# yuxng/PoseCNN

Hardware: NVIDIA H100
Metric: frames/sec on 640x480 RGB, 21 classes, batch 32 (VGG16 + Hough + ROI pose head) (higher is better)
Workload: dtype bf16 operands / fp32 accumulate (conv stack, 1x1 heads), fp16 operands / fp32 accumulate (fc6-fc8), fp32 / int32 elsewhere

## Files before the change

### posecnn_b200/csrc/conv_tc.cu

```cuda
#include <cuda.h>
#include <cuda_bf16.h>

#include <type_traits>

#include "common.cuh"
#include "tc_common.cuh"

namespace pcnn {
namespace convtc {

constexpr int kTileH = 8, kTileW = 16;
static_assert(kTileH * kTileW == kTileM, "pixel tile = two wgmma M blocks");
constexpr int kABytes = kTileM * kKC * 2;
constexpr int kConsumers = 256;
constexpr int kProducerWarp = kConsumers / 32;
constexpr int kThreadsConv = kConsumers + 128;
constexpr int kConsumerRegs = 232, kProducerRegs = 40;
constexpr int kThreadsRow = kConsumers + 32;
constexpr int kStageBytes = 16 * 1024;

struct ConvParams {
    int B, H, W, Cin, Cout;
    int taps, ksize;
    int tiles_h, tiles_w, n_tiles_n, total_tiles;
// ... 107 lines not shown
                    uint8_t* sa = smem + stage * Plan::kStage;
                    mbar_arrive_expect_tx(&full[stage], Plan::kStage);
                    tma_load_4d(sa, &map_in, &full[stage], c0, w0 + dx, h0 + dy, img);
                    tma_load_2d(sa + Plan::kABytesT, &map_w, &full[stage], tap * p.Cin + c0, n0);
                    if (++stage == Plan::kStages) { stage = 0; phase ^= 1; }
                }
            }
        }
    } else {
        setmaxnreg_inc<kConsumerRegs>();
        const int wg = warp >> 2, wq = warp & 3;
        const int row = wg * 64 + wq * 16 + (lane >> 2);
        float acc[kMB][BN / 2];
        int stage = 0, obuf = 0;
        uint32_t phase = 0;
        for (int tile = blockIdx.x; tile < p.total_tiles; tile += gridDim.x) {
            const int nt = tile % p.n_tiles_n;
            int rest = tile / p.n_tiles_n;
            const int tw = rest % p.tiles_w; rest /= p.tiles_w;
            const int th = rest % p.tiles_h;
            const int img = rest / p.tiles_h;
            const int h0 = th * p.tile_h, w0 = tw * p.tile_w, n0 = nt * BN;
            int prev = -1;
            for (int ks = 0; ks < ksteps; ks++) {
                mbar_wait(&full[stage], phase);
                const uint32_t sa = smem_u32(smem + stage * Plan::kStage);
                const uint64_t db = make_desc(sa + Plan::kABytesT);
#pragma unroll
                for (int h = 0; h < kMB; h++) acc_fence<BN / 2>(acc[h]);
                wgmma_fence();
#pragma unroll
                for (int h = 0; h < kMB; h++) {
                    const uint64_t da = make_desc(sa + (h * 2 + wg) * 64 * 128);
#pragma unroll
                    for (int k = 0; k < kKC / 16; k++)
                        wgmma<BN, 0, 0, 0>(acc[h], da + (uint64_t)(k * 2), db + (uint64_t)(k * 2), (ks | k) != 0);
                }
                wgmma_commit();
#pragma unroll
                for (int h = 0; h < kMB; h++) acc_fence<BN / 2>(acc[h]);
                if (prev >= 0) {
                    wgmma_wait<1>();
                    release(&empty[prev], lane);
                }
                prev = stage;
                if (++stage == Plan::kStages) { stage = 0; phase ^= 1; }
            }
            wgmma_wait<0>();
#pragma unroll
            for (int h = 0; h < kMB; h++) acc_fence<BN / 2>(acc[h]);
            release(&empty[prev], lane);
#pragma unroll
            for (int h = 0; h < kMB; h++) {
                if (h > 0 && h0 + 8 * h >= p.H) break;
#pragma unroll
                for (int g = 0; g < BN / 64; g++) {
                    if (threadIdx.x == 0) tma_store_wait_read<1>();
                    consumer_sync();
                    uint8_t* ob = out_stage + obuf * kStageBytes;
                    stage_rows(ob, acc[h] + g * 32, p.bias + n0 + g * 64, p.relu, row, lane & 3);
                    if (p.pool) {
                        consumer_sync();
                        pool_staged(ob, threadIdx.x);
                    }
                    fence_proxy_async();
                    consumer_sync();
                    if (threadIdx.x == 0) {
                        if (!p.pool) tma_store_4d(&map_out, ob, n0 + g * 64, w0, h0 + 8 * h, img);
                        else tma_store_4d(&map_out, ob, n0 + g * 64, w0 >> 1, (h0 >> 1) + 4 * h, img);
                        tma_store_commit();
                    }
                    obuf ^= 1;
                }
            }
        }
        if (threadIdx.x == 0) tma_store_wait_all();
    }
}

constexpr int kRowPx = 128, kPatchW = 130, kPatchH = 4;
constexpr int kPatchBytes = kPatchW * kPatchH * 128;
constexpr int kRowAStages = 2;

template <int BN, bool RESB>
struct RowPlan {
    static constexpr int kBBytes = BN * 128;
    static constexpr int kBStages = RESB ? 9 : 6;
    static constexpr int kBOff = kRowAStages * kPatchBytes;
    static constexpr int kOutOff = kBOff + kBStages * kBBytes;
    static constexpr int kOutBytes = RESB ? kStageBytes : 2 * kStageBytes;
    static constexpr int kBarOff = kOutOff + kOutBytes;
    static constexpr int kTotal = kBarOff + 256 + 1024;
};

template <int BN, bool RESB>
__global__ void __launch_bounds__(kThreadsRow, 1)
k_conv_row2(const __grid_constant__ CUtensorMap map_in , const __grid_constant__ CUtensorMap map_w,
            const __grid_constant__ CUtensorMap map_out ,
            const ConvParams p)
{
    using Plan = RowPlan<BN, RESB>;
    static_assert(BN == 64, "row mode: 64-channel N tiles");
    extern __shared__ uint8_t smem_raw[];
    uint8_t* smem = reinterpret_cast<uint8_t*>((reinterpret_cast<uintptr_t>(smem_raw) + 1023) & ~(uintptr_t)1023);
    uint8_t* sB = smem + Plan::kBOff;
    uint8_t* out_stage = smem + Plan::kOutOff;
    uint64_t* fullA = reinterpret_cast<uint64_t*>(smem + Plan::kBarOff);
    uint64_t* emptyA = fullA + kRowAStages;
    uint64_t* fullB = emptyA + kRowAStages;
    uint64_t* emptyB = fullB + Plan::kBStages;
    uint64_t* wbar = emptyB + Plan::kBStages;
    const int warp = threadIdx.x >> 5, lane = threadIdx.x & 31;
    const int kchunks = p.Cin / kKC;
    const int tile0 = RESB ? blockIdx.x / p.n_tiles_n : blockIdx.x;
    const int tstep = RESB ? gridDim.x / p.n_tiles_n : gridDim.x;
    const int tcount = RESB ? p.total_tiles / p.n_tiles_n : p.total_tiles;
    const int nt_fixed = blockIdx.x % p.n_tiles_n;
    if (warp == kProducerWarp && lane == 0) {
        asm volatile("prefetch.tensormap [%0];" ::"l"(&map_in) : "memory");
        asm volatile("prefetch.tensormap [%0];" ::"l"(&map_w) : "memory");
        asm volatile("prefetch.tensormap [%0];" ::"l"(&map_out) : "memory");
        for (int s = 0; s < kRowAStages; s++) { mbar_init(&fullA[s], 1); mbar_init(&emptyA[s], kConsumers / 32); }
        for (int s = 0; s < Plan::kBStages; s++) { mbar_init(&fullB[s], 1); mbar_init(&emptyB[s], kConsumers / 32); }
        mbar_init(wbar, 1);
        fence_barrier_init();
    }
    __syncthreads();

    if (warp == kProducerWarp) {
        if (elect_one()) {
            int sa = 0, sb = 0;
            uint32_t pa = 0, pb = 0;
            if (RESB) {
                mbar_arrive_expect_tx(wbar, 9 * Plan::kBBytes);
                for (int tap = 0; tap < 9; tap++)
                    tma_load_2d(sB + tap * Plan::kBBytes, &map_w, wbar, tap * p.Cin, nt_fixed * BN);
            }
            for (int tile = tile0; tile < tcount; tile += tstep) {
                const int nt = RESB ? nt_fixed : tile % p.n_tiles_n;
                int rest = RESB ? tile : tile / p.n_tiles_n;
                const int tw = rest % p.tiles_w; rest /= p.tiles_w;
                const int yp = rest % p.tiles_h;
                const int img = rest / p.tiles_h;
                const int y0 = 2 * yp, x0 = tw * kRowPx, n0 = nt * BN;
                for (int c = 0; c < kchunks; c++) {
                    mbar_wait(&emptyA[sa], pa ^ 1);
                    mbar_arrive_expect_tx(&fullA[sa], kPatchBytes);
                    tma_load_4d(smem + sa * kPatchBytes, &map_in, &fullA[sa], c * kKC, x0 - 1, y0 - 1, img);
                    if (++sa == kRowAStages) { sa = 0; pa ^= 1; }
                    if (!RESB) {
                        for (int tap = 0; tap < 9; tap++) {
                            mbar_wait(&emptyB[sb], pb ^ 1);
                            mbar_arrive_expect_tx(&fullB[sb], Plan::kBBytes);
                            tma_load_2d(sB + sb * Plan::kBBytes, &map_w, &fullB[sb], tap * p.Cin + c * kKC, n0);
                            if (++sb == Plan::kBStages) { sb = 0; pb ^= 1; }
                        }
                    }
                }
            }
        }
    } else {
        constexpr int kH = BN / 2;
        const int wg = warp >> 2, wq = warp & 3;
        const int row = wg * 64 + wq * 16 + (lane >> 2);
        float acc[2 * kH];
        int sa = 0, sb = 0, obuf = 0;
        uint32_t pa = 0, pb = 0;
        if (RESB) mbar_wait(wbar, 0);
        for (int tile = tile0; tile < tcount; tile += tstep) {
            const int nt = RESB ? nt_fixed : tile % p.n_tiles_n;
            int rest = RESB ? tile : tile / p.n_tiles_n;
            const int tw = rest % p.tiles_w; rest /= p.tiles_w;
            const int yp = rest % p.tiles_h;
            const int img = rest / p.tiles_h;
            const int y0 = 2 * yp, x0 = tw * kRowPx, n0 = nt * BN;
            for (int c = 0; c < kchunks; c++) {
                mbar_wait(&fullA[sa], pa);
                const uint32_t a_base = smem_u32(smem + sa * kPatchBytes) + wg * 64 * 128;
                if constexpr (RESB) {
                    acc_fence<2 * kH>(acc);
                    wgmma_fence();
#pragma unroll
                    for (int o = 0; o < 4; o++) {
                        const int rho = o == 0 ? 1 : (o == 1 ? 2 : (o == 2 ? 0 : 3));
#pragma unroll
                        for (int s3 = 0; s3 < 3; s3++) {
                            const uint64_t da = make_desc(a_base + (uint32_t)((rho * kPatchW + s3) * 128));
#pragma unroll
                            for (int j = 0; j < 2; j++) {
                                const int r = rho - j;
                                if (r < 0 || r > 2) continue;
                                const uint64_t db = make_desc(smem_u32(sB + (r * 3 + s3) * Plan::kBBytes));
#pragma unroll
                                for (int k = 0; k < kKC / 16; k++)
                                    wgmma<BN, 0, 0, 0>(acc + j * kH, da + (uint64_t)(k * 2), db + (uint64_t)(k * 2), (c | o | s3 | k) != 0);
                            }
                        }
                    }
                    wgmma_commit();
                    wgmma_wait<0>();
                    acc_fence<2 * kH>(acc);
                } else {
                    int prevb = -1;
                    for (int tap = 0; tap < 9; tap++) {
                        mbar_wait(&fullB[sb], pb);
                        const int r = tap / 3, s = tap - 3 * r;
                        const uint64_t db = make_desc(smem_u32(sB + sb * Plan::kBBytes));
                        acc_fence<2 * kH>(acc);
                        wgmma_fence();
#pragma unroll
                        for (int j = 0; j < 2; j++) {
                            const uint64_t da = make_desc(a_base + (uint32_t)(((r + j) * kPatchW + s) * 128));
#pragma unroll
                            for (int k = 0; k < kKC / 16; k++)
                                wgmma<BN, 0, 0, 0>(acc + j * kH, da + (uint64_t)(k * 2), db + (uint64_t)(k * 2), (c | tap | k) != 0);
                        }
                        wgmma_commit();
                        acc_fence<2 * kH>(acc);
                        if (prevb >= 0) {
                            wgmma_wait<1>();
                            release(&emptyB[prevb], lane);
                        }
                        prevb = sb;
                        if (++sb == Plan::kBStages) { sb = 0; pb ^= 1; }
                    }
                    wgmma_wait<0>();
                    acc_fence<2 * kH>(acc);
                    release(&emptyB[prevb], lane);
                }
                release(&emptyA[sa], lane);
                if (++sa == kRowAStages) { sa = 0; pa ^= 1; }
            }
            if (!p.pool) {
#pragma unroll
                for (int j = 0; j < 2; j++) {
#pragma unroll
                    for (int g = 0; g < BN / 64; g++) {
                        if (threadIdx.x == 0) { if (RESB) tma_store_wait_read<0>(); else tma_store_wait_read<1>(); }
                        consumer_sync();
                        uint8_t* ob = out_stage + (RESB ? 0 : obuf * kStageBytes);
                        stage_rows(ob, acc + j * kH + g * 32, p.bias + n0 + g * 64, p.relu, row, lane & 3);
                        fence_proxy_async();
                        consumer_sync();
                        if (threadIdx.x == 0) {
                            tma_store_4d(&map_out, ob, n0 + g * 64, x0, y0 + j, img);
                            tma_store_commit();
                        }
                        obuf ^= 1;
                    }
                }
            } else {
#pragma unroll
                for (int g = 0; g < BN / 64; g++) {
                    if (threadIdx.x == 0) tma_store_wait_read<1>();
                    consumer_sync();
                    uint8_t* ob = out_stage + obuf * (RESB ? kStageBytes / 2 : kStageBytes);
                    const float* a0 = acc + g * 32;
                    const float* a1 = acc + kH + g * 32;
                    const float* bias = p.bias + n0 + g * 64;
                    const int q = lane & 3;
#pragma unroll
                    for (int i = 0; i < 2; i++) {
                        const int r = row + 8 * i;
                        const int prow = r >> 1;
#pragma unroll
                        for (int jj = 0; jj < 8; jj++) {
                            const int c = 8 * jj + 2 * q;
                            float v0 = fmaxf(a0[4 * jj + 2 * i], a1[4 * jj + 2 * i]) + __ldg(bias + c);
                            float v1 = fmaxf(a0[4 * jj + 2 * i + 1], a1[4 * jj + 2 * i + 1]) + __ldg(bias + c + 1);
                            if (p.relu) { v0 = fmaxf(v0, 0.f); v1 = fmaxf(v1, 0.f); }
                            uint32_t pk = pack_bf16(v0, v1);
                            uint32_t o1 = __shfl_xor_sync(0xffffffffu, pk, 4);
                            __nv_bfloat162 m2 = __hmax2(*reinterpret_cast<__nv_bfloat162*>(&pk), *reinterpret_cast<__nv_bfloat162*>(&o1));
                            if ((lane & 4) == 0)
                                *reinterpret_cast<__nv_bfloat162*>(ob + prow * 128 + ((jj ^ (prow & 7)) << 4) + 4 * q) = m2;
                        }
                    }
                    fence_proxy_async();
                    consumer_sync();
                    if (threadIdx.x == 0) {
                        tma_store_4d(&map_out, ob, n0 + g * 64, x0 >> 1, y0 >> 1, img);
                        tma_store_commit();
                    }
                    obuf ^= 1;
                }
            }
        }
        if (threadIdx.x == 0) tma_store_wait_all();
    }
}

constexpr int kC1Stages = 6;
constexpr int kC1EpiGroups = 2, kC1BuildGroups = 4;
constexpr int kC1Threads = 128 * (kC1EpiGroups + kC1BuildGroups);
constexpr int kC1PatchWords = 10 * 16;
constexpr int kC1PatchOff = kC1Stages * kABytes + 64 * 128 + kC1EpiGroups * 2 * kStageBytes;
constexpr int kC1BarOff = kC1PatchOff + kC1BuildGroups * 2 * kC1PatchWords * 4;
constexpr int kC1Smem = kC1BarOff + 256 + 1024;

struct DepthIn { float d; };

__device__ __forceinline__ float depth_gray(float d)
{
    return __fmul_rn(fminf(fmaxf(__fdiv_rn(d, 2000.f), 0.f), 1.f), 255.f);
}

template <typename TIn>
__global__ void __launch_bounds__(kC1Threads, 1)
k_conv1_tc(const TIn* __restrict__ in, const __grid_constant__ CUtensorMap map_w, const __grid_constant__ CUtensorMap map_out,
           const ConvParams p, float m0, float m1, float m2)
{
    constexpr int BN = 64;
    extern __shared__ uint8_t smem_raw[];
    uint8_t* smem = reinterpret_cast<uint8_t*>((reinterpret_cast<uintptr_t>(smem_raw) + 1023) & ~(uintptr_t)1023);
    uint8_t* sb = smem + kC1Stages * kABytes;
    uint8_t* out_stage = sb + 64 * 128;
    uint64_t* full = reinterpret_cast<uint64_t*>(smem + kC1BarOff);
    uint64_t* empty = full + kC1Stages;
    uint64_t* wbar = empty + kC1Stages;
    const int warp = threadIdx.x >> 5, lane = threadIdx.x & 31;

    if (threadIdx.x == 0) {
        asm volatile("prefetch.tensormap [%0];" ::"l"(&map_w) : "memory");
        asm volatile("prefetch.tensormap [%0];" ::"l"(&map_out) : "memory");
        for (int s = 0; s < kC1Stages; s++) { mbar_init(&full[s], 4); mbar_init(&empty[s], 4); }
        mbar_init(wbar, 1);
        fence_barrier_init();
    }
    __syncthreads();

    if (warp >= 4 * kC1EpiGroups) {
        const int group = (threadIdx.x - 128 * kC1EpiGroups) >> 7;
        const int r = (threadIdx.x - 128 * kC1EpiGroups) & 127;
        const int hl = r >> 4, wl = r & 15;
        uint32_t* patch_base = reinterpret_cast<uint32_t*>(smem + kC1PatchOff);
        const bool fast_u8 = sizeof(TIn) == 1 && (p.W & 3) == 0 && (reinterpret_cast<uintptr_t>(in) & 3) == 0;
        int it = 0, lit = 0;
        for (int tile = blockIdx.x; tile < p.total_tiles; tile += gridDim.x, it++) {
            if (it % kC1BuildGroups != group) continue;
            const int stage = it % kC1Stages;
            const uint32_t phase = (it / kC1Stages) & 1;
            const int tw = tile % p.tiles_w;
            const int rest = tile / p.tiles_w;
            const int th = rest % p.tiles_h, img = rest / p.tiles_h;
            const int y = th * kTileH + hl, x = tw * kTileW + wl;
            constexpr int kInCh = std::is_same<TIn, DepthIn>::value ? 1 : 3;
            const TIn* base = in + (size_t)img * p.H * p.W * kInCh;
            float v[32];
            v[27] = 1.f; v[28] = 1.f;
#pragma unroll
            for (int k = 29; k < 32; k++) v[k] = 0.f;
            bool done = false;
            if constexpr (sizeof(TIn) == 1) {
                if (fast_u8) {
                    uint32_t* pw = patch_base + (group * 2 + (lit & 1)) * kC1PatchWords;
                    const int y0 = th * kTileH - 1, wq0 = 12 * tw - 1, row_words = (p.W * 3) >> 2;
                    const uint32_t* img32 = reinterpret_cast<const uint32_t*>(base);
                    for (int idx = r; idx < 140; idx += 128) {
                        const int prow = idx / 14, wi = idx - prow * 14;
                        const int yy = y0 + prow, wq = wq0 + wi;
                        uint32_t word = 0;
                        if (yy >= 0 && yy < p.H && wq >= 0 && wq < row_words) word = __ldg(img32 + (size_t)yy * row_words + wq);
                        pw[prow * 16 + wi] = word;
                    }
                    if (group == 0) asm volatile("bar.sync 3, 128;" ::: "memory");
                    else if (group == 1) asm volatile("bar.sync 4, 128;" ::: "memory");
                    else if (group == 2) asm volatile("bar.sync 5, 128;" ::: "memory");
                    else asm volatile("bar.sync 6, 128;" ::: "memory");
                    const int boff = 1 + 3 * wl, w0 = boff >> 2, o = boff & 3;
                    const uint32_t sel = (uint32_t)(o | ((o + 1) << 4) | ((o + 2) << 8) | ((o + 3) << 12));
                    const bool border = th == 0 || th * kTileH + kTileH + 1 > p.H || tw == 0 || tw * kTileW + kTileW + 1 > p.W;
// ... 203 lines not shown
        if (yy >= 0 && yy < H && xx >= 0 && xx < W) {
            if constexpr (std::is_same<TIn, DepthIn>::value)
                v = __fsub_rn(depth_gray(img[yy * W + xx].d), c == 0 ? m0 : (c == 1 ? m1 : m2));
            else
                v = (float)img[(yy * W + xx) * 3 + c] - (c == 0 ? m0 : (c == 1 ? m1 : m2));
        }
        patch[r][rem] = v;
    }
    __syncthreads();
    const int j = t & 7;
#pragma unroll
    for (int pass = 0; pass < kSeg / 32; pass++) {
        const int xl = pass * 32 + (t >> 3), x = x0 + xl;
        if (x >= W) break;
        __align__(16) __nv_bfloat16 v[8];
#pragma unroll
        for (int e = 0; e < 8; e++) {
            const int k = j * 8 + e;
            float val = 0.f;
            if (k < 27) {
                const int dy = k / 9, rem = k - dy * 9;
                val = patch[dy][xl * 3 + rem];
            }
            v[e] = __float2bfloat16_rn(val);
        }
        *reinterpret_cast<uint4*>(out + (((size_t)n * H + y) * W + x) * 64 + j * 8) = *reinterpret_cast<const uint4*>(v);
    }
}

__global__ void __launch_bounds__(256)
k_maxpool2x2_bf16(const __nv_bfloat16* __restrict__ in, __nv_bfloat16* __restrict__ out, int B, int H, int W, int C)
{
    const int Ho = H / 2, Wo = W / 2, cg = C / 8;
    const size_t total = (size_t)B * Ho * Wo * cg;
    for (size_t idx = (size_t)blockIdx.x * blockDim.x + threadIdx.x; idx < total; idx += (size_t)gridDim.x * blockDim.x) {
        const int g = (int)(idx % cg);
        size_t r = idx / cg;
        const int xo = (int)(r % Wo); r /= Wo;
        const int yo = (int)(r % Ho);
        const size_t n = r / Ho;
        const __nv_bfloat16* p0 = in + ((n * H + 2 * yo) * W + 2 * xo) * C + g * 8;
        uint4 a = __ldg(reinterpret_cast<const uint4*>(p0));
        uint4 b = __ldg(reinterpret_cast<const uint4*>(p0 + C));
        uint4 c = __ldg(reinterpret_cast<const uint4*>(p0 + (size_t)W * C));
        uint4 d = __ldg(reinterpret_cast<const uint4*>(p0 + (size_t)W * C + C));
        uint4 o;
        const __nv_bfloat162* pa = reinterpret_cast<const __nv_bfloat162*>(&a);
        const __nv_bfloat162* pb = reinterpret_cast<const __nv_bfloat162*>(&b);
        const __nv_bfloat162* pc = reinterpret_cast<const __nv_bfloat162*>(&c);
        const __nv_bfloat162* pd = reinterpret_cast<const __nv_bfloat162*>(&d);
        __nv_bfloat162* po = reinterpret_cast<__nv_bfloat162*>(&o);
#pragma unroll
        for (int k = 0; k < 4; k++) po[k] = __hmax2(__hmax2(pa[k], pb[k]), __hmax2(pc[k], pd[k]));
        *reinterpret_cast<uint4*>(out + ((n * Ho + yo) * Wo + xo) * C + g * 8) = o;
    }
}

static int make_map_nhwc(CUtensorMap* m, const void* ptr, int B, int H, int W, int C, int box_c, int box_w = kTileW, int box_h = kTileH)
{
    EncodeTiledFn enc = get_encode();
    if (!enc) { set_error("cuTensorMapEncodeTiled unavailable (driver too old?)"); return PCNN_E_CUDA; }
    cuuint64_t dims[4] = {(cuuint64_t)C, (cuuint64_t)W, (cuuint64_t)H, (cuuint64_t)B};
    cuuint64_t strides[3] = {(cuuint64_t)C * 2, (cuuint64_t)W * C * 2, (cuuint64_t)H * W * C * 2};
    cuuint32_t box[4] = {(cuuint32_t)box_c, (cuuint32_t)box_w, (cuuint32_t)box_h, 1};
    cuuint32_t es[4] = {1, 1, 1, 1};
    CUresult r = enc(m, CU_TENSOR_MAP_DATA_TYPE_BFLOAT16, 4, const_cast<void*>(ptr), dims, strides, box, es,
                     CU_TENSOR_MAP_INTERLEAVE_NONE, CU_TENSOR_MAP_SWIZZLE_128B, CU_TENSOR_MAP_L2_PROMOTION_L2_256B,
                     CU_TENSOR_MAP_FLOAT_OOB_FILL_NONE);
    if (r != CUDA_SUCCESS) { set_error("cuTensorMapEncodeTiled(NHWC %dx%dx%dx%d) failed: %d", B, H, W, C, (int)r); return PCNN_E_CUDA; }
    return PCNN_OK;
}

template <int BN, int BM = kTileM>
static int launch_conv(const CUtensorMap& mi, const CUtensorMap& mw, const CUtensorMap& mo, const ConvParams& p, int num_sms,
                       cudaStream_t st)
{
    using Plan = SmemPlan<BN, BM>;
    PCNN_SMEM_OPTIN((k_conv_tc<BN, BM>), Plan::kTotal, "conv_tc");
    int grid = p.total_tiles < num_sms ? p.total_tiles : num_sms;
    k_conv_tc<BN, BM><<<grid, kThreadsConv, Plan::kTotal, st>>>(mi, mw, mo, p);
    return check_launch("conv_tc");
}

template <int BN, bool RESB>
static int launch_conv_row2(const CUtensorMap& mi, const CUtensorMap& mw, const CUtensorMap& mo, const ConvParams& p, int num_sms,
                            cudaStream_t st)
{
    using Plan = RowPlan<BN, RESB>;
    PCNN_SMEM_OPTIN((k_conv_row2<BN, RESB>), Plan::kTotal, "conv_row2");
    int grid = p.total_tiles < num_sms ? p.total_tiles : num_sms;
    if (RESB) grid = grid / p.n_tiles_n * p.n_tiles_n;
    k_conv_row2<BN, RESB><<<grid, kThreadsRow, Plan::kTotal, st>>>(mi, mw, mo, p);
    return check_launch("conv_row2");
}

}
}

using namespace pcnn;
using namespace pcnn::convtc;

static int conv_bf16_tc_impl(const void* in, const void* weights, const float* bias, void* out, int B, int H, int W, int Cin,
                            int Cout, int ksize, int relu, int block_n, int pool, void* stream);

extern "C" int pcnn_conv_bf16_tc(const void* in, const void* weights, const float* bias, void* out, int B, int H, int W,
                                 int Cin, int Cout, int ksize, int relu, int block_n, void* stream)
{
    return conv_bf16_tc_impl(in, weights, bias, out, B, H, W, Cin, Cout, ksize, relu, block_n, 0, stream);
}

extern "C" int pcnn_conv_pool_bf16_tc(const void* in, const void* weights, const float* bias, void* out_pooled, int B, int H,
                                      int W, int Cin, int Cout, int ksize, int relu, int block_n, void* stream)
{
    PCNN_REQUIRE(H % 2 == 0 && W % 2 == 0, "conv_pool: needs even H, W (got %d x %d)", H, W);
    return conv_bf16_tc_impl(in, weights, bias, out_pooled, B, H, W, Cin, Cout, ksize, relu, block_n, 1, stream);
}

static int conv_bf16_tc_impl(const void* in, const void* weights, const float* bias, void* out, int B, int H, int W, int Cin,
                            int Cout, int ksize, int relu, int block_n, int pool, void* stream)
{
    PCNN_REQUIRE(in && weights && bias && out, "conv: NULL tensor pointer");
    PCNN_REQUIRE(ksize == 1 || ksize == 3, "conv: ksize must be 1 or 3 (got %d)", ksize);
    PCNN_REQUIRE(Cin % 64 == 0 && Cin >= 64, "conv: Cin must be a multiple of 64 (got %d)", Cin);
    PCNN_REQUIRE(Cout % 64 == 0 && Cout >= 64, "conv: Cout must be a multiple of 64 (got %d)", Cout);
    PCNN_REQUIRE(B >= 1 && H >= 1 && W >= 1, "conv: bad shape");
    int bn = block_n;
    if (bn == 0) bn = Cout % 256 == 0 && ksize * ksize * Cin >= 2304 ? 256 : (Cout % 128 == 0 ? 128 : 64);
    PCNN_REQUIRE((bn == 64 || bn == 128 || bn == 256) && Cout % bn == 0, "conv: block_n %d does not divide Cout %d", bn, Cout);
    int dev = 0, sms = kNumSMs;
    cudaGetDevice(&dev);
    cudaDeviceGetAttribute(&sms, cudaDevAttrMultiProcessorCount, dev);
    cudaStream_t st = (cudaStream_t)stream;
    CUtensorMap mi, mw, mo;
    int rc;
    const bool tile256 = block_n == 0 && ksize == 3 && Cin <= 128 && Cout == 128;
    if (block_n == 0 && ksize == 3 && Cin <= 128 && Cout == 64 && H % 2 == 0 && W >= kRowPx) {
        const bool resb = Cin == 64;
        bn = 64;
        rc = make_map_nhwc(&mi, in, B, H, W, Cin, kKC, kPatchW, kPatchH);
        if (rc) return rc;
        rc = make_map_weights(&mw, weights, 9 * Cin, Cout, bn);
        if (rc) return rc;
        rc = pool ? make_map_nhwc(&mo, out, B, H / 2, W / 2, Cout, 64, kRowPx / 2, 1) : make_map_nhwc(&mo, out, B, H, W, Cout, 64, kRowPx, 1);
        if (rc) return rc;
        ConvParams p;
        p.B = B; p.H = H; p.W = W; p.Cin = Cin; p.Cout = Cout; p.ksize = 3; p.taps = 9;
        p.tile_h = 2; p.tile_w = kRowPx;
        p.tiles_h = H / 2;
        p.tiles_w = (W + kRowPx - 1) / kRowPx;
        p.n_tiles_n = Cout / bn;
        p.total_tiles = B * p.tiles_h * p.tiles_w * p.n_tiles_n;
        p.relu = relu; p.pool = pool; p.bias = bias; p.kc_outer = 0;
        if (resb && p.total_tiles >= p.n_tiles_n) return launch_conv_row2<64, true>(mi, mw, mo, p, sms, st);
        return launch_conv_row2<64, false>(mi, mw, mo, p, sms, st);
    }
    int tile_h = kTileH, tile_w = kTileW;
    if (tile256) tile_h = 2 * kTileH;
    else if (!pool && ((H + 15) / 16) * ((W + 7) / 8) < ((H + 7) / 8) * ((W + 15) / 16)) { tile_h = 16; tile_w = 8; }
    rc = make_map_nhwc(&mi, in, B, H, W, Cin, kKC, tile_w, tile_h);
    if (rc) return rc;
    rc = make_map_weights(&mw, weights, ksize * ksize * Cin, Cout, bn);
    if (rc) return rc;
    rc = pool ? make_map_nhwc(&mo, out, B, H / 2, W / 2, Cout, 64, kTileW / 2, kTileH / 2)
              : make_map_nhwc(&mo, out, B, H, W, Cout, 64, tile_w, tile256 ? kTileH : tile_h);
    if (rc) return rc;
    ConvParams p;
    p.B = B; p.H = H; p.W = W; p.Cin = Cin; p.Cout = Cout;
    p.ksize = ksize; p.taps = ksize * ksize;
    p.tile_h = tile_h; p.tile_w = tile_w;
    p.tiles_h = (H + tile_h - 1) / tile_h;
    p.tiles_w = (W + tile_w - 1) / tile_w;
    p.n_tiles_n = Cout / bn;
    p.total_tiles = B * p.tiles_h * p.tiles_w * p.n_tiles_n;
    p.relu = relu;
    p.pool = pool;
    p.bias = bias;
    p.kc_outer = tile256 && H % 2 == 0 && W >= kRowPx;
    if (tile256) return launch_conv<128, 256>(mi, mw, mo, p, sms, st);
    if (bn == 256) return launch_conv<256>(mi, mw, mo, p, sms, st);
    if (bn == 128) return launch_conv<128>(mi, mw, mo, p, sms, st);
    return launch_conv<64>(mi, mw, mo, p, sms, st);
}

extern "C" int pcnn_conv3x3_small_cin(const float* in, const float* weights_hwio, const float* bias, void* out, int B, int H,
                                      int W, int Cin, int Cout, int relu, void* stream)
{
    PCNN_REQUIRE(in && weights_hwio && bias && out, "conv_small: NULL tensor pointer");
    PCNN_REQUIRE(Cin >= 1 && Cin <= 8 && Cout % 16 == 0 && Cout <= 128, "conv_small: needs Cin <= 8, Cout %% 16 == 0, Cout <= 128");
    size_t smem = sizeof(float) * (size_t)(9 * Cin + 1) * Cout;
    size_t total = (size_t)B * H * W * (Cout / 16);
    int blocks = (int)((total + 255) / 256 < (size_t)kNumSMs * 8 ? (total + 255) / 256 : (size_t)kNumSMs * 8);
    k_conv_small_cin<16><<<blocks, 256, smem, (cudaStream_t)stream>>>(in, weights_hwio, bias, (__nv_bfloat16*)out, B, H, W, Cin,
                                                                      Cout, relu);
    return check_launch("conv_small_cin");
}

extern "C" int pcnn_maxpool2x2_bf16(const void* in, void* out, int B, int H, int W, int C, void* stream)
{
    PCNN_REQUIRE(in && out, "maxpool: NULL tensor pointer");
    PCNN_REQUIRE(H % 2 == 0 && W % 2 == 0 && C % 8 == 0, "maxpool: needs even H, W and C %% 8 == 0 (got %d,%d,%d)", H, W, C);
    size_t total = (size_t)B * (H / 2) * (W / 2) * (C / 8);
    int blocks = (int)((total + 255) / 256 < (size_t)kNumSMs * 16 ? (total + 255) / 256 : (size_t)kNumSMs * 16);
    k_maxpool2x2_bf16<<<blocks, 256, 0, (cudaStream_t)stream>>>((const __nv_bfloat16*)in, (__nv_bfloat16*)out, B, H, W, C);
    return check_launch("maxpool2x2");
}

extern "C" int pcnn_im2col_c3(const void* in, int in_is_u8, const float* mean3_host, void* out_bf16, int B, int H, int W,
                              void* stream)
{
    PCNN_REQUIRE(in && out_bf16, "im2col: NULL tensor pointer");
    float m0 = 0.f, m1 = 0.f, m2 = 0.f;
    if (mean3_host) { m0 = mean3_host[0]; m1 = mean3_host[1]; m2 = mean3_host[2]; }
    PCNN_REQUIRE(H <= 65535 && B <= 65535, "im2col: image too tall for the launch grid");
    dim3 grid((W + 127) / 128, H, B);
    cudaStream_t st = (cudaStream_t)stream;
    if (in_is_u8)
        k_im2col_c3<unsigned char><<<grid, 256, 0, st>>>((const unsigned char*)in, (__nv_bfloat16*)out_bf16, H, W, m0, m1, m2);
    else
        k_im2col_c3<float><<<grid, 256, 0, st>>>((const float*)in, (__nv_bfloat16*)out_bf16, H, W, m0, m1, m2);
    return check_launch("im2col_c3");
}

extern "C" int pcnn_im2col_depth(const float* depth, const float* mean3_host, void* out_bf16, int B, int H, int W, void* stream)
{
    PCNN_REQUIRE(depth && out_bf16, "im2col_depth: NULL tensor pointer");
    PCNN_REQUIRE(B >= 1 && H >= 1 && W >= 1, "im2col_depth: bad shape (%d,%d,%d)", B, H, W);
    PCNN_REQUIRE(H <= 65535 && B <= 65535, "im2col_depth: image too tall for the launch grid");
    float m0 = 0.f, m1 = 0.f, m2 = 0.f;
    if (mean3_host) { m0 = mean3_host[0]; m1 = mean3_host[1]; m2 = mean3_host[2]; }
    dim3 grid((W + 127) / 128, H, B);
    k_im2col_c3<DepthIn><<<grid, 256, 0, (cudaStream_t)stream>>>((const DepthIn*)depth, (__nv_bfloat16*)out_bf16, H, W, m0, m1, m2);
    return check_launch("im2col_depth");
}

static int conv1_fused_impl(const void* in, int in_kind, const float* mean3_host, const void* weights_bf16,
                            const float* bias, void* out_bf16, int B, int H, int W, int relu, void* stream);

// ... 46 lines not shown
```

Before: 2887.

## Add swapped-operand row conv kernel with resident weights for Cin=64 layers

Replaces the resident-weight variant of the row conv kernel with a new kernel for Cin=64, Cout=64 3x3 convs. Weights become the wgmma A operand (M=64 output channels) and input pixels the N=128 operand. Two consumer warpgroups each take alternate tiles, with named barriers so their wgmma issue interleaves. The epilogue writes transposed output through half-row TMA stores, with an in-register 2x2 pool path. The goal is wider N per wgmma and overlap of one warpgroup's epilogue with the other's math. The cost is a more complex epilogue with 64-pixel stores and per-warpgroup serialization.

Result: faster. 2969, median of 6 (+2.8%).

```diff
diff --git a/posecnn_b200/csrc/conv_tc.cu b/posecnn_b200/csrc/conv_tc.cu
--- a/posecnn_b200/csrc/conv_tc.cu
+++ b/posecnn_b200/csrc/conv_tc.cu
@@ -213,24 +213,23 @@
 constexpr int kPatchBytes = kPatchW * kPatchH * 128;
 constexpr int kRowAStages = 2;
 
-template <int BN, bool RESB>
+template <int BN>
 struct RowPlan {
     static constexpr int kBBytes = BN * 128;
-    static constexpr int kBStages = RESB ? 9 : 6;
+    static constexpr int kBStages = 6;
     static constexpr int kBOff = kRowAStages * kPatchBytes;
     static constexpr int kOutOff = kBOff + kBStages * kBBytes;
-    static constexpr int kOutBytes = RESB ? kStageBytes : 2 * kStageBytes;
-    static constexpr int kBarOff = kOutOff + kOutBytes;
+    static constexpr int kBarOff = kOutOff + 2 * kStageBytes;
     static constexpr int kTotal = kBarOff + 256 + 1024;
 };
 
-template <int BN, bool RESB>
+template <int BN>
 __global__ void __launch_bounds__(kThreadsRow, 1)
 k_conv_row2(const __grid_constant__ CUtensorMap map_in , const __grid_constant__ CUtensorMap map_w,
             const __grid_constant__ CUtensorMap map_out ,
             const ConvParams p)
 {
-    using Plan = RowPlan<BN, RESB>;
+    using Plan = RowPlan<BN>;
     static_assert(BN == 64, "row mode: 64-channel N tiles");
     extern __shared__ uint8_t smem_raw[];
     uint8_t* smem = reinterpret_cast<uint8_t*>((reinterpret_cast<uintptr_t>(smem_raw) + 1023) & ~(uintptr_t)1023);
@@ -240,20 +239,14 @@
     uint64_t* emptyA = fullA + kRowAStages;
     uint64_t* fullB = emptyA + kRowAStages;
     uint64_t* emptyB = fullB + Plan::kBStages;
-    uint64_t* wbar = emptyB + Plan::kBStages;
     const int warp = threadIdx.x >> 5, lane = threadIdx.x & 31;
     const int kchunks = p.Cin / kKC;
-    const int tile0 = RESB ? blockIdx.x / p.n_tiles_n : blockIdx.x;
-    const int tstep = RESB ? gridDim.x / p.n_tiles_n : gridDim.x;
-    const int tcount = RESB ? p.total_tiles / p.n_tiles_n : p.total_tiles;
-    const int nt_fixed = blockIdx.x % p.n_tiles_n;
     if (warp == kProducerWarp && lane == 0) {
         asm volatile("prefetch.tensormap [%0];" ::"l"(&map_in) : "memory");
         asm volatile("prefetch.tensormap [%0];" ::"l"(&map_w) : "memory");
         asm volatile("prefetch.tensormap [%0];" ::"l"(&map_out) : "memory");
         for (int s = 0; s < kRowAStages; s++) { mbar_init(&fullA[s], 1); mbar_init(&emptyA[s], kConsumers / 32); }
         for (int s = 0; s < Plan::kBStages; s++) { mbar_init(&fullB[s], 1); mbar_init(&emptyB[s], kConsumers / 32); }
-        mbar_init(wbar, 1);
         fence_barrier_init();
     }
     __syncthreads();
@@ -262,14 +255,9 @@
         if (elect_one()) {
             int sa = 0, sb = 0;
             uint32_t pa = 0, pb = 0;
-            if (RESB) {
-                mbar_arrive_expect_tx(wbar, 9 * Plan::kBBytes);
-                for (int tap = 0; tap < 9; tap++)
-                    tma_load_2d(sB + tap * Plan::kBBytes, &map_w, wbar, tap * p.Cin, nt_fixed * BN);
-            }
-            for (int tile = tile0; tile < tcount; tile += tstep) {
-                const int nt = RESB ? nt_fixed : tile % p.n_tiles_n;
-                int rest = RESB ? tile : tile / p.n_tiles_n;
+            for (int tile = blockIdx.x; tile < p.total_tiles; tile += gridDim.x) {
+                const int nt = tile % p.n_tiles_n;
+                int rest = tile / p.n_tiles_n;
                 const int tw = rest % p.tiles_w; rest /= p.tiles_w;
                 const int yp = rest % p.tiles_h;
                 const int img = rest / p.tiles_h;
@@ -279,13 +267,11 @@
                     mbar_arrive_expect_tx(&fullA[sa], kPatchBytes);
                     tma_load_4d(smem + sa * kPatchBytes, &map_in, &fullA[sa], c * kKC, x0 - 1, y0 - 1, img);
                     if (++sa == kRowAStages) { sa = 0; pa ^= 1; }
-                    if (!RESB) {
-                        for (int tap = 0; tap < 9; tap++) {
-                            mbar_wait(&emptyB[sb], pb ^ 1);
-                            mbar_arrive_expect_tx(&fullB[sb], Plan::kBBytes);
-                            tma_load_2d(sB + sb * Plan::kBBytes, &map_w, &fullB[sb], tap * p.Cin + c * kKC, n0);
-                            if (++sb == Plan::kBStages) { sb = 0; pb ^= 1; }
-                        }
+                    for (int tap = 0; tap < 9; tap++) {
+                        mbar_wait(&emptyB[sb], pb ^ 1);
+                        mbar_arrive_expect_tx(&fullB[sb], Plan::kBBytes);
+                        tma_load_2d(sB + sb * Plan::kBBytes, &map_w, &fullB[sb], tap * p.Cin + c * kKC, n0);
+                        if (++sb == Plan::kBStages) { sb = 0; pb ^= 1; }
                     }
                 }
             }
@@ -297,10 +283,9 @@
         float acc[2 * kH];
         int sa = 0, sb = 0, obuf = 0;
         uint32_t pa = 0, pb = 0;
-        if (RESB) mbar_wait(wbar, 0);
-        for (int tile = tile0; tile < tcount; tile += tstep) {
-            const int nt = RESB ? nt_fixed : tile % p.n_tiles_n;
-            int rest = RESB ? tile : tile / p.n_tiles_n;
+        for (int tile = blockIdx.x; tile < p.total_tiles; tile += gridDim.x) {
+            const int nt = tile % p.n_tiles_n;
+            int rest = tile / p.n_tiles_n;
             const int tw = rest % p.tiles_w; rest /= p.tiles_w;
             const int yp = rest % p.tiles_h;
             const int img = rest / p.tiles_h;
@@ -308,57 +293,32 @@
             for (int c = 0; c < kchunks; c++) {
                 mbar_wait(&fullA[sa], pa);
                 const uint32_t a_base = smem_u32(smem + sa * kPatchBytes) + wg * 64 * 128;
-                if constexpr (RESB) {
+                int prevb = -1;
+                for (int tap = 0; tap < 9; tap++) {
+                    mbar_wait(&fullB[sb], pb);
+                    const int r = tap / 3, s = tap - 3 * r;
+                    const uint64_t db = make_desc(smem_u32(sB + sb * Plan::kBBytes));
                     acc_fence<2 * kH>(acc);
                     wgmma_fence();
 #pragma unroll
-                    for (int o = 0; o < 4; o++) {
-                        const int rho = o == 0 ? 1 : (o == 1 ? 2 : (o == 2 ? 0 : 3));
-#pragma unroll
-                        for (int s3 = 0; s3 < 3; s3++) {
-                            const uint64_t da = make_desc(a_base + (uint32_t)((rho * kPatchW + s3) * 128));
-#pragma unroll
-                            for (int j = 0; j < 2; j++) {
-                                const int r = rho - j;
-                                if (r < 0 || r > 2) continue;
-                                const uint64_t db = make_desc(smem_u32(sB + (r * 3 + s3) * Plan::kBBytes));
-#pragma unroll
-                                for (int k = 0; k < kKC / 16; k++)
-                                    wgmma<BN, 0, 0, 0>(acc + j * kH, da + (uint64_t)(k * 2), db + (uint64_t)(k * 2), (c | o | s3 | k) != 0);
-                            }
-                        }
+                    for (int j = 0; j < 2; j++) {
+                        const uint64_t da = make_desc(a_base + (uint32_t)(((r + j) * kPatchW + s) * 128));
+#pragma unroll
+                        for (int k = 0; k < kKC / 16; k++)
+                            wgmma<BN, 0, 0, 0>(acc + j * kH, da + (uint64_t)(k * 2), db + (uint64_t)(k * 2), (c | tap | k) != 0);
                     }
                     wgmma_commit();
-                    wgmma_wait<0>();
                     acc_fence<2 * kH>(acc);
-                } else {
-                    int prevb = -1;
-                    for (int tap = 0; tap < 9; tap++) {
-                        mbar_wait(&fullB[sb], pb);
-                        const int r = tap / 3, s = tap - 3 * r;
-                        const uint64_t db = make_desc(smem_u32(sB + sb * Plan::kBBytes));
-                        acc_fence<2 * kH>(acc);
-                        wgmma_fence();
-#pragma unroll
-                        for (int j = 0; j < 2; j++) {
-                            const uint64_t da = make_desc(a_base + (uint32_t)(((r + j) * kPatchW + s) * 128));
-#pragma unroll
-                            for (int k = 0; k < kKC / 16; k++)
-                                wgmma<BN, 0, 0, 0>(acc + j * kH, da + (uint64_t)(k * 2), db + (uint64_t)(k * 2), (c | tap | k) != 0);
-                        }
-                        wgmma_commit();
-                        acc_fence<2 * kH>(acc);
-                        if (prevb >= 0) {
-                            wgmma_wait<1>();
-                            release(&emptyB[prevb], lane);
-                        }
-                        prevb = sb;
-                        if (++sb == Plan::kBStages) { sb = 0; pb ^= 1; }
-                    }
-                    wgmma_wait<0>();
-                    acc_fence<2 * kH>(acc);
-                    release(&emptyB[prevb], lane);
-                }
+                    if (prevb >= 0) {
+                        wgmma_wait<1>();
+                        release(&emptyB[prevb], lane);
+                    }
+                    prevb = sb;
+                    if (++sb == Plan::kBStages) { sb = 0; pb ^= 1; }
+                }
+                wgmma_wait<0>();
+                acc_fence<2 * kH>(acc);
+                release(&emptyB[prevb], lane);
                 release(&emptyA[sa], lane);
                 if (++sa == kRowAStages) { sa = 0; pa ^= 1; }
             }
@@ -367,9 +327,9 @@
                 for (int j = 0; j < 2; j++) {
 #pragma unroll
                     for (int g = 0; g < BN / 64; g++) {
-                        if (threadIdx.x == 0) { if (RESB) tma_store_wait_read<0>(); else tma_store_wait_read<1>(); }
+                        if (threadIdx.x == 0) tma_store_wait_read<1>();
                         consumer_sync();
-                        uint8_t* ob = out_stage + (RESB ? 0 : obuf * kStageBytes);
+                        uint8_t* ob = out_stage + obuf * kStageBytes;
                         stage_rows(ob, acc + j * kH + g * 32, p.bias + n0 + g * 64, p.relu, row, lane & 3);
                         fence_proxy_async();
                         consumer_sync();
@@ -385,7 +345,7 @@
                 for (int g = 0; g < BN / 64; g++) {
                     if (threadIdx.x == 0) tma_store_wait_read<1>();
                     consumer_sync();
-                    uint8_t* ob = out_stage + obuf * (RESB ? kStageBytes / 2 : kStageBytes);
+                    uint8_t* ob = out_stage + obuf * kStageBytes;
                     const float* a0 = acc + g * 32;
                     const float* a1 = acc + kH + g * 32;
                     const float* bias = p.bias + n0 + g * 64;
@@ -418,6 +378,156 @@
             }
         }
         if (threadIdx.x == 0) tma_store_wait_all();
+    }
+}
+
+constexpr int kRowNWBytes = 64 * 128;
+constexpr int kRowNOutBytes = 64 * 128;
+constexpr int kRowNWOff = kRowAStages * kPatchBytes;
+constexpr int kRowNOutOff = kRowNWOff + 9 * kRowNWBytes;
+constexpr int kRowNBarOff = kRowNOutOff + 2 * kRowNOutBytes;
+constexpr int kRowNSmem = kRowNBarOff + 256 + 1024;
+
+__device__ __forceinline__ void bar_sync(int id, int n) { asm volatile("bar.sync %0, %1;" ::"r"(id), "r"(n) : "memory"); }
+__device__ __forceinline__ void bar_arrive(int id, int n) { asm volatile("bar.arrive %0, %1;" ::"r"(id), "r"(n) : "memory"); }
+
+__global__ void __launch_bounds__(kThreadsConv, 1)
+k_conv_rown(const __grid_constant__ CUtensorMap map_in , const __grid_constant__ CUtensorMap map_w,
+            const __grid_constant__ CUtensorMap map_out ,
+            const ConvParams p)
+{
+    extern __shared__ uint8_t smem_raw[];
+    uint8_t* smem = reinterpret_cast<uint8_t*>((reinterpret_cast<uintptr_t>(smem_raw) + 1023) & ~(uintptr_t)1023);
+    uint8_t* sW = smem + kRowNWOff;
+    uint64_t* fullA = reinterpret_cast<uint64_t*>(smem + kRowNBarOff);
+    uint64_t* emptyA = fullA + kRowAStages;
+    uint64_t* wbar = emptyA + kRowAStages;
+    const int warp = threadIdx.x >> 5, lane = threadIdx.x & 31;
+    if (warp == kProducerWarp && lane == 0) {
+        asm volatile("prefetch.tensormap [%0];" ::"l"(&map_in) : "memory");
+        asm volatile("prefetch.tensormap [%0];" ::"l"(&map_w) : "memory");
+        asm volatile("prefetch.tensormap [%0];" ::"l"(&map_out) : "memory");
+        for (int s = 0; s < kRowAStages; s++) { mbar_init(&fullA[s], 1); mbar_init(&emptyA[s], 4); }
+        mbar_init(wbar, 1);
+        fence_barrier_init();
+    }
+    __syncthreads();
+
+    if (warp >= kProducerWarp) {
+        setmaxnreg_dec<kProducerRegs>();
+        if (warp == kProducerWarp && elect_one()) {
+            mbar_arrive_expect_tx(wbar, 9 * kRowNWBytes);
+            for (int tap = 0; tap < 9; tap++) tma_load_2d(sW + tap * kRowNWBytes, &map_w, wbar, tap * kKC, 0);
+            int it = 0;
+#pragma unroll 1
+            for (int tile = blockIdx.x; tile < p.total_tiles; tile += gridDim.x, it++) {
+                const int tw = tile % p.tiles_w, rest = tile / p.tiles_w;
+                const int yp = rest % p.tiles_h, img = rest / p.tiles_h;
+                const int s = it & 1;
+                mbar_wait(&emptyA[s], ((it >> 1) & 1) ^ 1);
+                mbar_arrive_expect_tx(&fullA[s], kPatchBytes);
+                tma_load_4d(smem + s * kPatchBytes, &map_in, &fullA[s], 0, tw * kRowPx - 1, 2 * yp - 1, img);
+            }
+        }
+    } else {
+        setmaxnreg_inc<kConsumerRegs>();
+        const int wg = warp >> 2, wq = warp & 3, q = lane & 3;
+        const int co = wq * 16 + (lane >> 2);
+        const float bias0 = __ldg(p.bias + co), bias1 = __ldg(p.bias + co + 8);
+        const bool issuer = (threadIdx.x & 127) == 0;
+        uint8_t* ob = smem + kRowNOutOff + wg * kRowNOutBytes;
+        const uint32_t w_base = smem_u32(sW);
+        const uint32_t b_base = smem_u32(smem + wg * kPatchBytes);
+        float acc[2][64];
+        mbar_wait(wbar, 0);
+        int it = wg;
+        for (int tile = blockIdx.x + wg * gridDim.x; tile < p.total_tiles; tile += 2 * gridDim.x, it += 2) {
+            const int tw = tile % p.tiles_w, rest = tile / p.tiles_w;
+            const int yp = rest % p.tiles_h, img = rest / p.tiles_h;
+            const int y0 = 2 * yp, x0 = tw * kRowPx;
+            if (it > 0) bar_sync(3 + wg, 256);
+            mbar_wait(&fullA[wg], (it >> 1) & 1);
+            acc_fence<64>(acc[0]);
+            acc_fence<64>(acc[1]);
+            wgmma_fence();
+#pragma unroll
+            for (int j = 0; j < 2; j++) {
+#pragma unroll
+                for (int ri = 0; ri < 3; ri++) {
+                    const int r = j == 0 ? (ri + 1) % 3 : ri;
+#pragma unroll
+                    for (int s = 0; s < 3; s++) {
+                        const uint64_t da = make_desc(w_base + (uint32_t)((r * 3 + s) * kRowNWBytes));
+                        const uint64_t db = make_desc(b_base + (uint32_t)(((r + j) * kPatchW + s) * 128));
+#pragma unroll
+                        for (int k = 0; k < kKC / 16; k++)
+                            wgmma<128, 0, 0, 0>(acc[j], da + (uint64_t)(k * 2), db + (uint64_t)(k * 2), (ri | s | k) != 0);
+                    }
+                }
+            }
+            wgmma_commit();
+            if (tile + gridDim.x < p.total_tiles) bar_arrive(3 + (wg ^ 1), 256);
+            wgmma_wait<0>();
+            acc_fence<64>(acc[0]);
+            acc_fence<64>(acc[1]);
+            release(&emptyA[wg], lane);
+            if (p.pool) {
+                if (issuer) tma_store_wait_read<0>();
+                bar_sync(1 + wg, 128);
+#pragma unroll
+                for (int jn = 0; jn < 16; jn++) {
+                    const int pp = 4 * jn + q;
+                    float v[2][2];
+#pragma unroll
+                    for (int e = 0; e < 2; e++) {
+                        v[e][0] = fmaxf(acc[0][4 * jn + e], acc[1][4 * jn + e]) + bias0;
+                        v[e][1] = fmaxf(acc[0][4 * jn + 2 + e], acc[1][4 * jn + 2 + e]) + bias1;
+                        if (p.relu) { v[e][0] = fmaxf(v[e][0], 0.f); v[e][1] = fmaxf(v[e][1], 0.f); }
+                    }
+                    uint32_t pe = pack_bf16(v[0][0], v[0][1]), po = pack_bf16(v[1][0], v[1][1]);
+                    __nv_bfloat162 m2 = __hmax2(*reinterpret_cast<__nv_bfloat162*>(&pe), *reinterpret_cast<__nv_bfloat162*>(&po));
+                    uint8_t* rowp = ob + pp * 128 + (lane >> 2) * 2;
+                    *reinterpret_cast<__nv_bfloat16*>(rowp + (((2 * wq) ^ (pp & 7)) << 4)) = m2.x;
+                    *reinterpret_cast<__nv_bfloat16*>(rowp + (((2 * wq + 1) ^ (pp & 7)) << 4)) = m2.y;
+                }
+                fence_proxy_async();
+                bar_sync(1 + wg, 128);
+                if (issuer) {
+                    tma_store_4d(&map_out, ob, 0, x0 >> 1, y0 >> 1, img);
+                    tma_store_commit();
+                }
+            } else {
+#pragma unroll
+                for (int j = 0; j < 2; j++) {
+#pragma unroll
+                    for (int h = 0; h < 2; h++) {
+                        if (x0 + 64 * h >= p.W) continue;
+                        if (issuer) tma_store_wait_read<0>();
+                        bar_sync(1 + wg, 128);
+#pragma unroll
+                        for (int jl = 0; jl < 8; jl++) {
+                            const int jn = 8 * h + jl;
+#pragma unroll
+                            for (int e = 0; e < 2; e++) {
+                                const int pl = 8 * jl + 2 * q + e;
+                                float v0 = acc[j][4 * jn + e] + bias0, v1 = acc[j][4 * jn + 2 + e] + bias1;
+                                if (p.relu) { v0 = fmaxf(v0, 0.f); v1 = fmaxf(v1, 0.f); }
+                                uint8_t* rowp = ob + pl * 128 + (lane >> 2) * 2;
+                                *reinterpret_cast<__nv_bfloat16*>(rowp + (((2 * wq) ^ (pl & 7)) << 4)) = __float2bfloat16_rn(v0);
+                                *reinterpret_cast<__nv_bfloat16*>(rowp + (((2 * wq + 1) ^ (pl & 7)) << 4)) = __float2bfloat16_rn(v1);
+                            }
+                        }
+                        fence_proxy_async();
+                        bar_sync(1 + wg, 128);
+                        if (issuer) {
+                            tma_store_4d(&map_out, ob, 0, x0 + 64 * h, y0 + j, img);
+                            tma_store_commit();
+                        }
+                    }
+                }
+            }
+        }
+        if (issuer) tma_store_wait_all();
     }
 }
 
@@ -787,16 +897,24 @@
     return check_launch("conv_tc");
 }
 
-template <int BN, bool RESB>
+template <int BN>
 static int launch_conv_row2(const CUtensorMap& mi, const CUtensorMap& mw, const CUtensorMap& mo, const ConvParams& p, int num_sms,
                             cudaStream_t st)
 {
-    using Plan = RowPlan<BN, RESB>;
-    PCNN_SMEM_OPTIN((k_conv_row2<BN, RESB>), Plan::kTotal, "conv_row2");
+    using Plan = RowPlan<BN>;
+    PCNN_SMEM_OPTIN((k_conv_row2<BN>), Plan::kTotal, "conv_row2");
     int grid = p.total_tiles < num_sms ? p.total_tiles : num_sms;
-    if (RESB) grid = grid / p.n_tiles_n * p.n_tiles_n;
-    k_conv_row2<BN, RESB><<<grid, kThreadsRow, Plan::kTotal, st>>>(mi, mw, mo, p);
+    k_conv_row2<BN><<<grid, kThreadsRow, Plan::kTotal, st>>>(mi, mw, mo, p);
     return check_launch("conv_row2");
+}
+
+static int launch_conv_rown(const CUtensorMap& mi, const CUtensorMap& mw, const CUtensorMap& mo, const ConvParams& p, int num_sms,
+                            cudaStream_t st)
+{
+    PCNN_SMEM_OPTIN(k_conv_rown, kRowNSmem, "conv_rown");
+    int grid = p.total_tiles < num_sms ? p.total_tiles : num_sms;
+    k_conv_rown<<<grid, kThreadsConv, kRowNSmem, st>>>(mi, mw, mo, p);
+    return check_launch("conv_rown");
 }
 
 }
@@ -840,13 +958,14 @@
     int rc;
     const bool tile256 = block_n == 0 && ksize == 3 && Cin <= 128 && Cout == 128;
     if (block_n == 0 && ksize == 3 && Cin <= 128 && Cout == 64 && H % 2 == 0 && W >= kRowPx) {
-        const bool resb = Cin == 64;
+        const bool rown = Cin == 64;
         bn = 64;
         rc = make_map_nhwc(&mi, in, B, H, W, Cin, kKC, kPatchW, kPatchH);
         if (rc) return rc;
         rc = make_map_weights(&mw, weights, 9 * Cin, Cout, bn);
         if (rc) return rc;
-        rc = pool ? make_map_nhwc(&mo, out, B, H / 2, W / 2, Cout, 64, kRowPx / 2, 1) : make_map_nhwc(&mo, out, B, H, W, Cout, 64, kRowPx, 1);
+        const int box_w = pool || rown ? kRowPx / 2 : kRowPx;
+        rc = pool ? make_map_nhwc(&mo, out, B, H / 2, W / 2, Cout, 64, box_w, 1) : make_map_nhwc(&mo, out, B, H, W, Cout, 64, box_w, 1);
         if (rc) return rc;
         ConvParams p;
         p.B = B; p.H = H; p.W = W; p.Cin = Cin; p.Cout = Cout; p.ksize = 3; p.taps = 9;
@@ -856,8 +975,8 @@
         p.n_tiles_n = Cout / bn;
         p.total_tiles = B * p.tiles_h * p.tiles_w * p.n_tiles_n;
         p.relu = relu; p.pool = pool; p.bias = bias; p.kc_outer = 0;
-        if (resb && p.total_tiles >= p.n_tiles_n) return launch_conv_row2<64, true>(mi, mw, mo, p, sms, st);
-        return launch_conv_row2<64, false>(mi, mw, mo, p, sms, st);
+        if (rown) return launch_conv_rown(mi, mw, mo, p, sms, st);
+        return launch_conv_row2<64>(mi, mw, mo, p, sms, st);
     }
     int tile_h = kTileH, tile_w = kTileW;
     if (tile256) tile_h = 2 * kTileH;
```
